# javad-jahangiri-iau/Detecting_Cyber_Attacks_with_Distilled_Large_Language_Models_in_Distributed_Networks

Hardware: AMD Instinct MI355X
Metric: batches/sec/client (DistilBERT seq128 bs32) + aggregated F1 after 1 FedAvg round, 1/2/4/8 MI355X (higher is better)
Workload: dtype bf16; 1 GPU; model=DistilBERT-base (6 layers) + Linear(768,2) DDoSClassifier, global_batch=32, seq_len=128, parallelism=fedavg1 (1 client/GPU)

## Files before the change

csrc/kernels/gemm.hip:

```cpp
#include "common.h"
#include "adam_epi.h"

#include <cstdlib>
#include <cstring>

namespace {

#include "adam_common.h"
#include "attn_s128.h"

enum Epi : int {
  EPI_BF16 = 0,
  EPI_BIAS = 1,
  EPI_BIAS_GELU = 2,
  EPI_GELU_BWD = 3,
  EPI_ADD = 4,
  EPI_F32 = 5,
  EPI_LN = 6,
  EPI_LN_BWD = 7,
  EPI_LN2 = 8,
  EPI_LN2_BWD = 9,
  EPI_F32P = 10,
};
constexpr bool epi_f32(int e) { return e == EPI_F32 || e == EPI_F32P; }

struct GemmParams {
  const bf16_t* A;
  const bf16_t* B;
  void* C;
  int M, N, K;
  int lda, ldb, ldc;
  const float* bias;
  bf16_t* aux;
  int ldaux;
  const bf16_t* res;
  int ldres;
  int k_split;
// ... 38 lines not shown
  }
}
#else
#define FD_STAMP(i) do {} while (0)
DEV void stamp_hwid() {}
#endif

DEV void tile_coords(int lid, int tiles_m, int tiles_n, int gm, int& tm, int& tn) {
  const int per_group = gm * tiles_n;
  const int group = lid / per_group;
  const int first_m = group * gm;
  const int rows = min(gm, tiles_m - first_m);
  const int in_group = lid - group * per_group;
  tm = first_m + in_group % rows;
  tn = in_group / rows;
}

typedef __attribute__((address_space(3))) void lds_void;
typedef __attribute__((address_space(1))) const void gbl_void;

#ifndef FD_GLDS_ASM
#define FD_GLDS_ASM 1
#endif
DEV void glds16(const void* src, char* lds) {
#if FD_GLDS_ASM
  const uint32_t dst = __builtin_amdgcn_readfirstlane(
      (uint32_t)(uintptr_t)(lds_void*)lds);
  uint32_t keep;
  asm volatile("s_mov_b32 %0, m0\n\ts_mov_b32 m0, %2\n\ts_nop 0\n\tglobal_load_lds_dwordx4 %1, off\n\ts_mov_b32 m0, %0"
               : "=&s"(keep) : "v"(src), "s"(dst) : "memory");
#else
  __builtin_amdgcn_global_load_lds((gbl_void*)src, (lds_void*)lds, 16, 0, 0);
#endif
}

template <int W>
DEV int fk(int k) {
  if constexpr (W == 128) return ((k & 3) | ((k >> 1) & 4)) << 1;
  else return (((k >> 1) & 1) | ((k >> 2) & 2)) << 1;
}

DEV int ksw(int r) { return (r >> 1) & 7; }

template <int ROWS, bool KMAJ, int NWAVES, int BK = BKT>
struct Operand {
  static_assert(BK == BKT || (!KMAJ && BK == 32), "32-deep slots: MN-major images only");
  static constexpr int BYTES = ROWS * BK * 2;
  static constexpr int PER_WAVE = BYTES / 1024 / NWAVES;
  static constexpr int SUB = (ROWS % 128 == 0) ? 128 : 64;
  static constexpr int SUB_BYTES = BK * SUB * 2;
  static constexpr int SUB_CH = SUB / 8;

  DEV static void stage(const bf16_t* base, int ld, int row0, int k0, int lim, char* lds, int wid, int lane) {
    const char* sbase = reinterpret_cast<const char*>(KMAJ ? base + k0 : base + (size_t)k0 * ld + row0);
#pragma unroll
    for (int i = 0; i < PER_WAVE; ++i) {
      const int piece = wid * PER_WAVE + i;
      const int pos = piece * 64 + lane;
      uint32_t off;
      if constexpr (KMAJ) {
        const int r = pos >> 3, c = (pos & 7) ^ ksw(r);
        const int gr = min(row0 + r, lim - 1);
        off = (uint32_t)(gr * ld + c * 8) * 2u;
      } else {
        const int sub = pos / (SUB_BYTES / 16), lp = pos % (SUB_BYTES / 16);
        const int k = lp / SUB_CH, c = (lp % SUB_CH) ^ fk<SUB>(k);
// ... 758 lines not shown
  if constexpr (MAXN >= 3) { if (n >= 3) { wait_vm<3 * L>(); return; } }
  if constexpr (MAXN >= 2) { if (n >= 2) { wait_vm<2 * L>(); return; } }
  if constexpr (MAXN >= 1) { if (n >= 1) { wait_vm<L>(); return; } }
  wait_vm<0>();
}

template <int BM, int BN, bool AK, bool BKM, int EPI, int WM, int WN, int S, int BK = BKT>
struct GemmCfg {
  static constexpr int NW = WM * WN;
  using OA = Operand<BM, AK, NW, BK>;
  using OB = Operand<BN, BKM, NW, BK>;
  static constexpr int BUF = OA::BYTES + OB::BYTES;
  static constexpr int EPI_BYTES = EpiTraits<EPI, BM, BN>::DIRECT ? (BM / WM) * (BN * 4 + 16)
                                                                   : EpiTraits<EPI, BM, BN>::BYTES;
  static constexpr int SMEM = S * BUF > EPI_BYTES ? S * BUF : EPI_BYTES;
  static constexpr bool VALID = SMEM <= LDS_MAX && !EpiTraits<EPI, BM, BN>::DIRECT &&
                                (!EpiTraits<EPI, BM, BN>::LN || EpiTraits<EPI, BM, BN>::F32S) &&
                                (BKM || BN % 64 == 0) &&
                                (AK || BM % 64 == 0) &&
                                (BM / WM) % 16 == 0 && (BN / WN) % 16 == 0 &&
                                OA::PER_WAVE * NW * 1024 == OA::BYTES && OB::PER_WAVE * NW * 1024 == OB::BYTES;
};

struct GemmGroup {
  GemmParams q;
  int ntiles0;
  int ntiles;
};

#ifndef FD_GEMM_SCHED
#define FD_GEMM_SCHED 1
#endif

template <int BM, int BN, bool AK, bool BKM, int EPI, int WM, int WN, int S, int BK = BKT, bool WT = false>
DEV void gemm_tile_at(const GemmParams& p, int tm, int tn, char* smem) {
  const int tm_ = tm, tn_ = tn;
  using G = GemmCfg<BM, BN, AK, BKM, EPI, WM, WN, S, BK>;
  constexpr int KS = BK / 32;
  using OA = typename G::OA;
  using OB = typename G::OB;
  constexpr int NW = G::NW;
  constexpr int TM = BM / WM, TN = BN / WN;
  constexpr int MI = TM / 16, NI = TN / 16;
  constexpr int BUF = G::BUF;
  constexpr int L = OA::PER_WAVE + OB::PER_WAVE;
  static_assert(S >= 2 && S <= 6, "ring depth");
  static_assert((S - 2) * L <= 63, "vmcnt is 6 bits");
  constexpr bool SCHED = FD_GEMM_SCHED;

  const int tid = threadIdx.x, lane = tid & 63;
  const int wid = __builtin_amdgcn_readfirstlane(tid >> 6);
  const int wr = wid / WN, wc = wid % WN;
  const int m0 = tm * BM, n0 = tn * BN;
  const int kbeg = blockIdx.z * p.k_split;
  const int nk = p.k_split / BK;

  f32x4 acc[MI][NI];
#pragma unroll
  for (int i = 0; i < MI; ++i)
#pragma unroll
    for (int j = 0; j < NI; ++j) acc[i][j] = f32x4{0.f, 0.f, 0.f, 0.f};

  auto issue = [&](int t) {
    char* b = smem + (t % S) * BUF;
    OA::stage(p.A, p.lda, m0, kbeg + t * BK, p.M, b, wid, lane);
    OB::stage(p.B, p.ldb, n0, kbeg + t * BK, p.N, b + OA::BYTES, wid, lane);
  };
// ... 19 lines not shown
    }
  };
  auto read_frags = [&](const char* cur) {
#pragma unroll
    for (int i = 0; i < MI; ++i) a0[i] = OA::frag(cur, wr * TM + i * 16, 0, lane);
#pragma unroll
    for (int j = 0; j < NI; ++j) b0[j] = OB::frag(cur + OA::BYTES, wc * TN + j * 16, 0, lane);
    if constexpr (KS == 2) {
#pragma unroll
      for (int i = 0; i < MI; ++i) a1[i] = OA::frag(cur, wr * TM + i * 16, 1, lane);
#pragma unroll
      for (int j = 0; j < NI; ++j) b1[j] = OB::frag(cur + OA::BYTES, wc * TN + j * 16, 1, lane);
    }
  };
  auto mfmas = [&]() {
    if constexpr (!SCHED) __builtin_amdgcn_s_setprio(1);
#pragma unroll
    for (int i = 0; i < MI; ++i)
#pragma unroll
      for (int j = 0; j < NI; ++j) acc[i][j] = mfma16(b0[j], a0[i], acc[i][j]);
    if constexpr (KS == 2) {
#pragma unroll
      for (int i = 0; i < MI; ++i)
#pragma unroll
        for (int j = 0; j < NI; ++j) acc[i][j] = mfma16(b1[j], a1[i], acc[i][j]);
    }
    if constexpr (!SCHED) __builtin_amdgcn_s_setprio(0);
  };

  constexpr bool LNPF = EpiTraits<EPI, BM, BN>::LN && S >= 6 && BN == 64 && (BM * BN * 2 / 1024) % NW == 0 &&
                        2 * BUF >= LN_DMA_MISC + 3072;
  const bool lnpf = LNPF && nk % S == 0 && nk >= S && p.M % 4 == 0 && !(p.diag & (1 | 128));
  int e_ops = 0;
  if constexpr (S < 6) {
#pragma unroll
    for (int t = 0; t < S - 1; ++t)
      if (t < nk) issue(t);

    for (int kt = 0; kt < nk; ++kt) {
      wait_tiles<L, S - 2>(min(S - 2, nk - 1 - kt));
      __builtin_amdgcn_s_barrier();
      asm volatile("" ::: "memory");
      if (FD_GEMM_STAMPS && kt == 0) FD_STAMP(1);
      if (kt + S - 1 < nk && !(p.diag & 1)) issue(kt + S - 1);
      read_frags(smem + (kt % S) * BUF);
      mfmas();
      sum_a();
      if constexpr (SCHED) sched_ktile<(MI * (AK ? 1 : 2) + NI * (BKM ? 1 : 2)) * KS / 2, MI * NI * KS / 2>();
    }
  } else {
#pragma unroll
    for (int t = 0; t < S - 2; ++t)
      if (t < nk) issue(t);

    for (int kt = 0; kt < nk; kt += 2) {
      const int issued = min(nk, S - 2 + kt);
      const int need = min(kt + 2, nk);
      if (LNPF && lnpf && kt == nk - 2) {
        wait_ops(e_ops);
      } else {
        wait_tiles<L, S - 4>(min(S - 4, max(0, issued - need)));
      }
      __builtin_amdgcn_s_barrier();
      asm volatile("" ::: "memory");
      if (FD_GEMM_STAMPS && kt == 0) FD_STAMP(1);
      if (!(p.diag & 1)) {
        if (kt + S - 2 < nk) issue(kt + S - 2);
// ... 68 lines not shown
        }
      }
      __syncthreads();
      f32_epilogue<TM, BN, 64 * NW, EPI == EPI_F32P>(p, smem, LDC, m0 + band * TM, n0, tid);
    }
  } else if constexpr (EpiTraits<EPI, BM, BN>::LN2) {
    static_assert((BM == 128 || BM == 256) && BN == 128 && WM == 4 && TN == 64, "two-K-half LayerNorm tile");
    constexpr bool BWD2 = EPI == EPI_LN2_BWD;
    const int s = p.ln2_half, tn_ln = 2 * tn + s, pair = tm * (p.N / BN) + tn;
    const uint32_t tag =
        (uint32_t)__hip_atomic_load(p.ln.cnt, __ATOMIC_RELAXED, __HIP_MEMORY_SCOPE_AGENT) * FD_LN_XSITES + p.ln.xsite + 1u;
    ln2_send<MI, NI>(p, acc, pair, s, wr, wc, lane, tag);
    const auto pre = ln_prefetch<BM, 64, BWD2, 64 * NW>(p, tm, tn_ln, tid);
    ln2_recv<MI, NI>(p, acc, pair, s, wc, wr, lane, tag);
    if (wc == s) ln_park<BM, 64, TM, TN, BWD2>(p, acc, smem, tn_ln * 64, wr, 0, lane);
    ln_finish<BM, 64, BWD2, 64 * NW>(p, smem, tm, tn_ln, lane, tid, pre);
  } else if constexpr (EpiTraits<EPI, BM, BN>::LN) {
    if (LNPF && lnpf) {
      wait_vm<0>();
      __syncthreads();
      const auto pre = ln_from_lds<BM, BN, EPI == EPI_LN_BWD, 64 * NW>(p, tm, tn, tid, smem);
      ln_epilogue<BM, BN, TM, TN, EPI == EPI_LN_BWD, 64 * NW>(p, acc, smem + 2 * BUF, tm, tn, wr, wc, lane, tid, pre);
    } else {
      const auto pre = ln_prefetch<BM, BN, EPI == EPI_LN_BWD, 64 * NW>(p, tm, tn, tid);
      __syncthreads();
      ln_epilogue<BM, BN, TM, TN, EPI == EPI_LN_BWD, 64 * NW>(p, acc, smem, tm, tn, wr, wc, lane, tid, pre);
    }
  } else {
    __syncthreads();
    staged_epilogue<BM, BN, TM, TN, EPI, 64 * NW, WT>(p, acc, smem, m0, n0, wr, wc, lane, tid);
  }
}

template <int BM, int BN, bool AK, bool BKM, int EPI, int WM, int WN, int S, int BK = BKT>
DEV void gemm_tile(const GemmParams& p, int bid, char* smem) {
  int tm, tn;
  tile_coords(bid, (p.M + BM - 1) / BM, p.N / BN, p.group_m, tm, tn);
  gemm_tile_at<BM, BN, AK, BKM, EPI, WM, WN, S, BK>(p, tm, tn, smem);
}

template <int BM, int BN, bool AK, bool BKM, int EPI, int WM, int WN, int S>
__global__ __launch_bounds__(64 * WM * WN, 2) void gemm_kernel(GemmParams p0, GemmGroup grp) {
  using G = GemmCfg<BM, BN, AK, BKM, EPI, WM, WN, S>;
  __shared__ __attribute__((aligned(1024))) char smem[G::SMEM];
  FD_STAMP(0);
  stamp_hwid();
  int bid = xcd_remap(blockIdx.x, grp.ntiles);
  const bool second = bid >= grp.ntiles0;
  const GemmParams& p = second ? grp.q : p0;
  if (second) bid -= grp.ntiles0;
  gemm_tile<BM, BN, AK, BKM, EPI, WM, WN, S>(p, bid, smem);
#if FD_GEMM_STAMPS
  __syncthreads();
  FD_STAMP(5);
#endif
}

struct QkvAttnSync {
  uint64_t* flags;
  const int* cnt;
  int* err;
  int xsite;
  int ntiles, tiles_n;
};
constexpr int QA_BM = 128, QA_BN = 192, QA_NW = 8;
using QaCfg = GemmCfg<QA_BM, QA_BN, true, true, EPI_BIAS, 2, 4, 2>;
static_assert(QaCfg::VALID && QaCfg::NW == QA_NW && QaCfg::SMEM >= ATT_FWD_SMEM, "fused QKV + attention tile");

__global__ __launch_bounds__(64 * QA_NW, 2) void gemm_attn_fwd_kernel(GemmParams p, AttnArgs a, QkvAttnSync q) {
  __shared__ __attribute__((aligned(1024))) char smem[QaCfg::SMEM];
  const uint32_t tag =
// ... 311 lines not shown
  const int lid = xcd_remap(blockIdx.x, gridDim.x);
  const int pair = lid >> 1, s = lid & 1, tiles_n2 = p.N / 128;
  GemmParams q = p;
  const int kh = p.K / 2;
  q.A = p.A + (size_t)s * kh;
  q.B = BKM ? p.B + (size_t)s * kh : p.B + (size_t)s * kh * p.ldb;
  q.k_split = kh;
  q.ln2_half = s;
  gemm_tile_at<BM, 128, true, BKM, EPI, 4, 2, S>(q, pair / tiles_n2, pair % tiles_n2, smem);
#if FD_GEMM_STAMPS
  __syncthreads();
  FD_STAMP(5);
#endif
}

constexpr int DWB_MAXP = 32;
using DwProb = FdDwProb;
struct DwBatch {
  DwProb pr[DWB_MAXP];
  int n, K, ntiles, group_m;
  int diag;
  const int* step;
  float lr, b1, b2, eps, wd;
  int decoupled;
  FdLrSched sched;
  float mu;
  FdAdamRest rest;
  int mixed;
  int cls_tiles[3], cls_off[3], cls_pad[3];
};

constexpr int DWB_HBM = 256, DWB_HBN = 128, DWB_HWM = 4, DWB_HWN = 2;

template <int BM, int BN, int WM, int WN, int S, int BK, bool MIX = false, bool PROX = false>
DEV void dwb_tile(const DwBatch& bt, int lid, char* smem) {
  constexpr int EPI = PROX ? EPI_F32P : EPI_F32;
  int i = 0;
  while (i + 1 < bt.n && lid >= bt.pr[i + 1].tile0) ++i;
  const DwProb& q = bt.pr[i];
  GemmParams p{};
  p.A = q.A; p.B = q.B; p.C = q.C;
  const int K = q.K > 0 ? q.K : bt.K;
  p.M = q.M; p.N = q.N; p.K = K;
  p.lda = q.M; p.ldb = q.N; p.ldc = q.N;
  p.k_split = K;
  p.group_m = bt.group_m;
  p.diag = bt.diag;
  p.out = q.C;
  p.accumulate = q.accumulate;
  p.acol = q.bias;
  if (q.p) {
    p.adam.p = q.p; p.adam.m = q.m; p.adam.v = q.v; p.adam.sh = q.sh; p.adam.step = bt.step;
    p.adam.lr = bt.lr; p.adam.b1 = bt.b1; p.adam.b2 = bt.b2; p.adam.eps = bt.eps; p.adam.wd = q.wd;
    p.adam.decoupled = bt.decoupled;
    if constexpr (PROX) {
      p.adam.mu = bt.mu;
      p.adam.anchor = q.anchor;
    }
    if (bt.sched.kind != 0)
      p.adam.lr = __int_as_float(
          __builtin_amdgcn_readfirstlane(__float_as_int(adam_lr_at(bt.lr, bt.sched, bt.step[0]))));
    if (q.bias && bt.rest.p) {
      const ptrdiff_t off = q.bias - bt.rest.g;
      p.acol_p = bt.rest.p + off; p.acol_m = bt.rest.m + off; p.acol_v = bt.rest.v + off;
      p.acol_sh = bt.rest.sh ? bt.rest.sh + off : nullptr;
      p.acol_wd = q.bias_wd;
      if constexpr (PROX) p.acol_a = bt.rest.anchor ? bt.rest.anchor + off : nullptr;
    }
  }
  if constexpr (MIX) {
    if (q.half) {
      gemm_tile<DWB_HBM, DWB_HBN, false, false, EPI, DWB_HWM, DWB_HWN, S, BK>(p, lid - q.tile0, smem);
      return;
    }
  }
  gemm_tile<BM, BN, false, false, EPI, WM, WN, S, BK>(p, lid - q.tile0, smem);
}

DEV int dwb_mixed_lid(const DwBatch& bt, int b) {
  const int x = b % 8;
  int j = b / 8, c = 0;
  while (c < 2 && j >= bt.cls_pad[c]) {
    j -= bt.cls_pad[c];
    ++c;
  }
  if (j >= bt.cls_pad[c]) return -1;
  const int t = x * bt.cls_pad[c] + j;
  return t < bt.cls_tiles[c] ? bt.cls_off[c] + t : -1;
}

constexpr int DWB_RUNS_LDS = 4096;
template <int NT, bool PROX>
DEV void dwb_rest(const DwBatch& bt, int rb, char* smem) {
  const FdAdamRest& r = bt.rest;
  float lr_t, ss, inv;
  adam_bias_corr(bt.step, bt.lr, bt.sched, bt.b1, bt.b2, lr_t, ss, inv);
  AdamArgs a{};
  a.step = bt.step; a.lr = lr_t; a.b1 = bt.b1; a.b2 = bt.b2; a.eps = bt.eps;
  a.mu = PROX ? bt.mu : 0.f;
  if (rb < r.flat_blocks) {
    a.p = r.p; a.g = r.g; a.m = r.m; a.v = r.v; a.shadow = reinterpret_cast<bf16_t*>(r.sh);
    a.anchor = r.anchor;
    a.wd = bt.wd; a.decoupled = bt.decoupled;
    a.runs = r.runs; a.nruns = r.nruns; a.n4 = r.n4;
    a.run_wd = r.run_wd;
    if (r.runs && 3 * r.nruns <= DWB_RUNS_LDS) {
      long long* rl = reinterpret_cast<long long*>(smem);
      for (int i = threadIdx.x; i < 3 * r.nruns; i += NT) rl[i] = r.runs[i];
      __syncthreads();
// ... 25 lines not shown
        if (v0 + u * stride >= r.n4) continue;
        const long long i = idx[u];
        float pp[4] = {p4[u].x, p4[u].y, p4[u].z, p4[u].w}, gg[4] = {g4[u].x, g4[u].y, g4[u].z, g4[u].w};
        float mm[4] = {m4[u].x, m4[u].y, m4[u].z, m4[u].w}, vv[4] = {v4[u].x, v4[u].y, v4[u].z, v4[u].w};
        adam_math4(a, wd[u], pp, gg, mm, vv, a4[u], ss, inv);
        st_nt(reinterpret_cast<float4*>(a.p) + i, make_float4(pp[0], pp[1], pp[2], pp[3]));
        st_nt(reinterpret_cast<float4*>(a.m) + i, make_float4(mm[0], mm[1], mm[2], mm[3]));
        st_nt(reinterpret_cast<float4*>(a.v) + i, make_float4(vv[0], vv[1], vv[2], vv[3]));
        if (a.shadow)
          reinterpret_cast<uint2*>(a.shadow)[i] = make_uint2(pack_bf2(pp[0], pp[1]), pack_bf2(pp[2], pp[3]));
      }
    }
    return;
  }
  if (!r.ever) return;
  a.p = r.p + r.woff; a.g = r.g + r.woff; a.m = r.m + r.woff; a.v = r.v + r.woff;
  a.shadow = r.sh ? reinterpret_cast<bf16_t*>(r.sh) + r.woff : nullptr;
  a.anchor = r.anchor ? r.anchor + r.woff : nullptr;
  a.wd = r.wwd; a.decoupled = bt.decoupled;
  a.touched = r.ever; a.now = r.now;
  const int lane = threadIdx.x & 63;
  const int nwaves = r.row_blocks * (NT / 64);
  for (int r0 = ((rb - r.flat_blocks) * (NT / 64) + (int)(threadIdx.x >> 6)) * 16; r0 < r.wrows; r0 += nwaves * 16)
    adam_rows16(a, r0, r.wrows, r.wrow4, lane, ss, inv);
}

template <int BM, int BN, int WM, int WN, int S, int BK, bool MIX>
constexpr int dwb_smem() {
  using G = GemmCfg<BM, BN, false, false, EPI_F32, WM, WN, S, BK>;
  using H = GemmCfg<DWB_HBM, DWB_HBN, false, false, EPI_F32, DWB_HWM, DWB_HWN, S, BK>;
  return MIX && H::SMEM > G::SMEM ? H::SMEM : G::SMEM;
}

template <int BM, int BN, int WM, int WN, int S, int BK = BKT, bool MIX = false, bool PROX = false>
__global__ __launch_bounds__(64 * WM * WN, 2) void gemm_dw_batch_kernel(DwBatch bt) {
  constexpr int SMEM = dwb_smem<BM, BN, WM, WN, S, BK, MIX>();
  static_assert(SMEM <= LDS_MAX, "LDS");
  static_assert(!MIX || (BM == DWB_HBM && WM * WN == DWB_HWM * DWB_HWN), "mixed tiles share the block shape");
  __shared__ __attribute__((aligned(1024))) char smem[SMEM];
  const int nrest = bt.rest.flat_blocks + bt.rest.row_blocks;
  int bid = blockIdx.x;
  if (bt.rest.first) {
    if (bid < nrest) {
      dwb_rest<64 * WM * WN, PROX>(bt, bid, smem);
      return;
    }
    bid -= nrest;
  } else {
    const int nblk = MIX && bt.mixed ? 8 * (bt.cls_pad[0] + bt.cls_pad[1] + bt.cls_pad[2]) : bt.ntiles;
    if (bid >= nblk) {
      dwb_rest<64 * WM * WN, PROX>(bt, bid - nblk, smem);
      return;
    }
  }
  if constexpr (MIX) {
    if (bt.mixed) {
      const int lid = dwb_mixed_lid(bt, bid);
      if (lid >= 0) dwb_tile<BM, BN, WM, WN, S, BK, true, PROX>(bt, lid, smem);
      return;
    }
  }
  dwb_tile<BM, BN, WM, WN, S, BK, false, PROX>(bt, xcd_remap(bid, bt.ntiles), smem);
}

__global__ __launch_bounds__(256) void splitk_reduce_kernel(const float* __restrict__ slabs, float* __restrict__ out,
                                                            long long n4, long long stride, int splits,
                                                            int accumulate) {
  for (long long i = blockIdx.x * 256ll + threadIdx.x; i < n4; i += (long long)gridDim.x * 256) {
    float4 s = accumulate ? reinterpret_cast<float4*>(out)[i] : make_float4(0.f, 0.f, 0.f, 0.f);
    for (int z = 0; z < splits; ++z) {
      const float4 v = reinterpret_cast<const float4*>(slabs + z * stride)[i];
      s.x += v.x; s.y += v.y; s.z += v.z; s.w += v.w;
    }
    reinterpret_cast<float4*>(out)[i] = s;
  }
}

constexpr int RED_MAXJ = 16;
struct ReduceJob {
  const float* slabs;
  float* out;
  long long n4, stride;
  int splits, accumulate;
};
struct ReduceBatch {
  ReduceJob j[RED_MAXJ];
  int start[RED_MAXJ + 1];
  int n;
};

__global__ __launch_bounds__(256) void splitk_reduce_batched_kernel(ReduceBatch rb) {
  int ji = 0;
  while (ji + 1 < rb.n && (int)blockIdx.x >= rb.start[ji + 1]) ++ji;
  const ReduceJob& jb = rb.j[ji];
  const int b0 = rb.start[ji], nb = rb.start[ji + 1] - b0;
// ... 411 lines not shown
  const int id = dw2_cfg(M0, N0, M1, N1);
  static const int diag = [] { const char* e = getenv("FD_GEMM_DIAG"); return e ? atoi(e) : 0; }();
  GemmParams p[2]{};
  const void* As[2] = {A0, A1};
  const void* Bs[2] = {B0, B1};
  float* Cs[2] = {C0, C1};
  const int Ms[2] = {M0, M1}, Ns[2] = {N0, N1};
  const long long panel = (long long)CFGS[id].bm * K * 2;
  const int gm = (int)std::max(1ll, std::min(16ll, (2ll << 20) / panel));
  for (int i = 0; i < 2; ++i) {
    p[i].A = (const bf16_t*)As[i]; p[i].B = (const bf16_t*)Bs[i]; p[i].C = Cs[i];
    p[i].M = Ms[i]; p[i].N = Ns[i]; p[i].K = K; p[i].lda = Ms[i]; p[i].ldb = Ns[i]; p[i].ldc = Ns[i];
    p[i].group_m = gm; p[i].diag = diag;
  }
  const int splits = fd_gemm_dw2_splits(M0, N0, M1, N1, K);
  if (splits <= 0) return 6;
  return dw_launch(p, 2, id, splits, K, workspace, workspace_elems, accumulate, adams, defer, splits_out, st);
}

bool dwb_launch_cfg(int id, DwBatch& bt, hipStream_t st, bool dry) {
  auto go = [&](auto kern, int bm, int bn, int threads) {
    for (int i = 0; i < bt.n; ++i)
      if (bt.pr[i].M % bm || bt.pr[i].N % (bt.pr[i].half ? DWB_HBN : bn)) return false;
    int t = 0;
    for (int i = 0; i < bt.n; ++i) {
      bt.pr[i].tile0 = t;
      t += (bt.pr[i].M / bm) * (bt.pr[i].N / (bt.pr[i].half ? DWB_HBN : bn));
    }
    bt.ntiles = t;
    const int nblk = bt.mixed ? 8 * (bt.cls_pad[0] + bt.cls_pad[1] + bt.cls_pad[2]) : t;
    if (!dry) hipLaunchKernelGGL(kern, dim3(nblk + bt.rest.flat_blocks + bt.rest.row_blocks), dim3(threads), 0, st, bt);
    return true;
  };
  if (bt.mixed && id != 11) return false;
  if (bt.mu != 0.f) {
    switch (id) {
      case 1: return go(gemm_dw_batch_kernel<128, 128, 2, 2, 2, BKT, false, true>, 128, 128, 256);
      case 8: return go(gemm_dw_batch_kernel<128, 64, 2, 2, 2, BKT, false, true>, 128, 64, 256);
      case 11: return go(gemm_dw_batch_kernel<256, 256, 2, 4, 2, BKT, true, true>, 256, 256, 512);
    }
    return false;
  }
  switch (id) {
    case 1: return go(gemm_dw_batch_kernel<128, 128, 2, 2, 2>, 128, 128, 256);
    case 8: return go(gemm_dw_batch_kernel<128, 64, 2, 2, 2>, 128, 64, 256);
    case 11: return go(gemm_dw_batch_kernel<256, 256, 2, 4, 2, BKT, true>, 256, 256, 512);
  }
  return false;
}

int g_dwb_mix = -1;
long long g_dwb_mixed_launches = 0;

int dwb_cus() {
  static const int cus = [] {
    int dev = 0, n = 0;
    if (hipGetDevice(&dev) != hipSuccess || hipDeviceGetAttribute(&n, hipDeviceAttributeMultiprocessorCount, dev) !=
                                                 hipSuccess)
      n = 0;
    return n > 0 ? n : 256;
  }();
  return cus;
}

bool plan_dwb_mix(DwBatch& bt, int mode) {
  if (mode <= 0 || bt.n < 2) return false;
  const int cus = dwb_cus();
  int kmax = 0;
  for (int i = 0; i < bt.n; ++i) kmax = std::max(kmax, bt.pr[i].K > 0 ? bt.pr[i].K : bt.K);
  int cls[DWB_MAXP], tiles[DWB_MAXP], L = 0, Sh = 0, nlong = 0;
  for (int i = 0; i < bt.n; ++i) {
    const DwProb& q = bt.pr[i];
    if (q.M % 256 || q.N % 256) return false;
    const int k = q.K > 0 ? q.K : bt.K;
    tiles[i] = (q.M / 256) * (q.N / 256);
    cls[i] = 8 * k <= kmax ? 2 : 0;
    if (cls[i] == 0) { L += tiles[i]; ++nlong; } else Sh += tiles[i];
  }
  if (nlong < 2) return false;
// ... 70 lines not shown
    if (!hyper || !step || !rest->g || !rest->m || !rest->v || (rest->nruns > 0) != (rest->runs != nullptr) ||
        rest->n4 < 0 || (rest->ever && (rest->wrows <= 0 || rest->wrow4 <= 0 || rest->woff % 4)))
      return 7;
    if ((rest->run_wd && !rest->runs) || (rest->ever && rest->wwd != 0.f && hyper[5] == 0.f)) return 8;
    bt.rest = *rest;
    bt.rest.flat_blocks = rest->n4 > 0 ? (int)std::min<long long>(128, (rest->n4 + 2047) / 2048) : 0;
    bt.rest.row_blocks = rest->ever ? std::min(128, (rest->wrows + 127) / 128) : 0;
    static const int first = [] { const char* e = getenv("FD_DW_REST_FIRST"); return e ? atoi(e) : 1; }();
    bt.rest.first = first;
    if (first) {
      const int pad = (8 - (bt.rest.flat_blocks + bt.rest.row_blocks) % 8) % 8;
      bt.rest.row_blocks += pad;
    }
  }
  bt.n = n;
  bt.K = K;
  static const int diag = [] { const char* e = getenv("FD_GEMM_DIAG"); return e ? atoi(e) : 0; }();
  bt.diag = diag;
  for (int i = 0; i < n; ++i) {
    bt.pr[i] = probs[i];
    if (!probs[i].A || !probs[i].B || (!probs[i].C && !probs[i].p) || probs[i].M <= 0 || probs[i].N <= 0) return 2;
    if (probs[i].K < 0 || probs[i].K % BKT) return 5;
    if (probs[i].p && (!probs[i].m || !probs[i].v || !step || !hyper)) return 3;
  }
  if (hyper) {
    bt.step = step;
    bt.lr = hyper[0]; bt.b1 = hyper[1]; bt.b2 = hyper[2]; bt.eps = hyper[3]; bt.wd = hyper[4];
    bt.decoupled = hyper[5] != 0.f;
    if (sched) bt.sched = *sched;
  }
  int id = cfg;
  if (id < 0) {
    static const int env = [] { const char* e = getenv("FD_GEMM_DWB_CFG"); return e ? atoi(e) : -1; }();
    id = env >= 0 ? env : 11;
  }
  bt.group_m = 64;
  static const int gm_env = [] { const char* e = getenv("FD_DWB_GROUP_M"); return e ? atoi(e) : 0; }();
  if (gm_env > 0) bt.group_m = gm_env;
  if (g_dwb_mix < 0) {
    const char* e = getenv("FD_DWB_MIX");
    g_dwb_mix = e ? atoi(e) : 1;
  }
  if (id == 11 && plan_dwb_mix(bt, g_dwb_mix) && !dwb_launch_cfg(id, bt, st, true)) {
    bt.mixed = 0;
    for (int i = 0; i < n; ++i) bt.pr[i] = probs[i];
  }
  if (bt.mixed) ++g_dwb_mixed_launches;
  if (!dwb_launch_cfg(id, bt, st, true)) {
    id = 8;
    if (!dwb_launch_cfg(id, bt, st, true)) return 4;
  }
  dwb_launch_cfg(id, bt, st, false);
  return 0;
}

int fd_splitk_reduce_batched(int n, const float* const* slabs, float* const* outs, const long long* numel,
                             const int* splits, const int* accumulate, hipStream_t st) {
  for (int base = 0; base < n; base += RED_MAXJ) {
    ReduceBatch rb{};
    rb.n = std::min(RED_MAXJ, n - base);
    int blocks = 0;
    for (int i = 0; i < rb.n; ++i) {
      const int k = base + i;
      if (numel[k] % 4 || splits[k] < 1) return 1;
      rb.j[i] = ReduceJob{slabs[k], outs[k], numel[k] / 4, numel[k], splits[k], accumulate[k]};
      rb.start[i] = blocks;
      blocks += (int)std::min<long long>((numel[k] / 4 + 1023) / 1024, 1024);
    }
    rb.start[rb.n] = blocks;
    hipLaunchKernelGGL(splitk_reduce_batched_kernel, dim3(blocks), dim3(256), 0, st, rb);
  }
  return 0;
}


long long fd_gemm_dwb_mixed_launches() { return g_dwb_mixed_launches; }
// ... 88 lines not shown
```

Measured before the change: 653.3 batches/s (sum over clients; bs32 x seq128).

## Add phased half-buffer pipelined main loop for 256x256 weight-gradient batch GEMM

Adds a new main-loop schedule for the 256x256 batched dW GEMM (config 13, now the default). Each K tile is split into four phases that read fragment quadrants and refill 16 KiB half-buffers as soon as their reads retire, with one counted vmcnt wait per tile and staggered barriers between wave rows. It also uses scalar-base global-to-LDS loads. The goal is to overlap DMA with MFMA work inside a two-slot ring without draining the pipeline. In exchange it adds more barriers per tile, a compile-time plan header with static checks, and a host simulator to verify RAW/WAR ordering.

```diff
diff --git a/csrc/host_check/dwb_phase_plan_check.cpp b/csrc/host_check/dwb_phase_plan_check.cpp
--- /dev/null
+++ b/csrc/host_check/dwb_phase_plan_check.cpp
@@ -0,0 +1,130 @@
+#include <cstdio>
+#include <deque>
+#include <vector>
+
+#include "../kernels/dwb_phase_plan.h"
+
+using namespace dwb_plan;
+
+namespace {
+
+constexpr int BIG = 1 << 30;
+enum Mode { STEADY, DRAIN, LAST };
+
+struct Group {
+  int interval = 0;
+  std::deque<int> fifo;
+  void barrier() { ++interval; }
+};
+
+struct Sim {
+  int nk;
+  std::vector<int> issue[2], retired[2], read_done[2];
+  int errors = 0;
+  explicit Sim(int nk_) : nk(nk_) {
+    for (int g = 0; g < 2; ++g) {
+      issue[g].assign(nk * HALVES, -1);
+      retired[g].assign(nk * HALVES, BIG);
+      read_done[g].assign(nk * HALVES, -1);
+    }
+  }
+  void fail(const char* what, int t, int h, int g) {
+    if (errors++ < 8) std::printf("  nk %d: %s (tile %d half %d group %d)\n", nk, what, t, h, g);
+  }
+  void stage(Group& G, int g, int t, int h) {
+    if (issue[g][t * HALVES + h] >= 0) fail("half-buffer staged twice", t, h, g);
+    for (int op = 0; op < OPS_PER_HALF; ++op) G.fifo.push_back(t * HALVES + h);
+    issue[g][t * HALVES + h] = G.interval;
+  }
+  void wait(Group& G, int g, int n) {
+    while ((int)G.fifo.size() > n) {
+      retired[g][G.fifo.front()] = G.interval;
+      G.fifo.pop_front();
+    }
+  }
+  void tile(Group& G, int g, int t, Mode mode) {
+    for (int p = 0; p < PHASES; ++p) {
+      const Phase& ph = PLAN[p];
+      for (int h = 0; h < HALVES; ++h)
+        if ((halves_of(ph.reads) >> h) & 1u) read_done[g][t * HALVES + h] = G.interval + 1;
+      for (int h = 0; h < HALVES; ++h)
+        if ((halves_of(ph.reads) >> h) & 1u) read_at.push_back({t * HALVES + h, g, G.interval});
+      if (mode != LAST)
+        for (int h = 0; h < HALVES; ++h)
+          if ((ph.stage_prev >> h) & 1u) stage(G, g, t + 1, h);
+      if (mode == STEADY)
+        for (int h = 0; h < HALVES; ++h)
+          if ((ph.stage >> h) & 1u) stage(G, g, t + 2, h);
+      if (ph.vmcnt >= 0 && mode != LAST) wait(G, g, mode == STEADY ? ph.vmcnt : 0);
+      G.barrier();
+      G.barrier();
+    }
+  }
+  struct Read { int id, g, interval; };
+  std::vector<Read> read_at;
+
+  int run_group(int g, bool stagger) {
+    Group G;
+    for (int h = 0; h < HALVES; ++h) stage(G, g, 0, h);
+    for (int h = 0; h < HALVES; ++h)
+      if ((own_halves() >> h) & 1u) stage(G, g, 1, h);
+    wait(G, g, PROLOGUE_VMCNT);
+    G.barrier();
+    if (stagger && g == 1) G.barrier();
+    int t = 0;
+    for (; t + 3 < nk; t += 2) {
+      tile(G, g, t, STEADY);
+      tile(G, g, t + 1, STEADY);
+    }
+    if (nk - t == 3) {
+      tile(G, g, t, STEADY);
+      tile(G, g, t + 1, DRAIN);
+      tile(G, g, t + 2, LAST);
+    } else {
+      tile(G, g, t, DRAIN);
+      tile(G, g, t + 1, LAST);
+    }
+    if (stagger && g == 0) G.barrier();
+    if (!G.fifo.empty()) fail("DMA still in flight at the epilogue", -1, -1, g);
+    return G.interval;
+  }
+  bool run(bool stagger) {
+    const int b0 = run_group(0, stagger), b1 = run_group(1, stagger);
+    if (b0 != b1 || b0 != 1 + BARRIERS_PER_TILE * nk + (stagger ? 1 : 0)) fail("barrier counts differ", -1, -1, 0);
+    for (const Read& r : read_at) {
+      const int t = r.id / HALVES, h = r.id % HALVES;
+      for (int g = 0; g < 2; ++g) {
+        if (issue[g][r.id] < 0) fail("read of a half-buffer that was never staged", t, h, g);
+        if (r.interval <= retired[g][r.id]) fail("RAW: read not behind the barrier after the retiring wait", t, h, r.g);
+      }
+    }
+    for (int id = 2 * HALVES; id < nk * HALVES; ++id)
+      for (int gi = 0; gi < 2; ++gi)
+        for (int gr = 0; gr < 2; ++gr)
+          if (issue[gi][id] <= read_done[gr][id - 2 * HALVES]) fail("WAR: refill not behind the reads' barrier", id / HALVES, id % HALVES, gi);
+    for (int t = 0; t < nk; ++t)
+      for (int h = 0; h < HALVES; ++h)
+        for (int g = 0; g < 2; ++g)
+          if (read_done[g][t * HALVES + h] < 0) fail("half-buffer never read", t, h, g);
+    return errors == 0;
+  }
+};
+
+}
+
+int main() {
+  bool ok = true;
+  const int nks[] = {2, 3, 4, 5, 6, 7, 8, 41, 42};
+  for (int nk : nks)
+    for (int stagger = 0; stagger < 2; ++stagger) {
+      Sim s(nk);
+      if (!s.run(stagger != 0)) {
+        std::printf("nk %d stagger %d: FAILED\n", nk, stagger);
+        ok = false;
+      }
+    }
+  std::printf("steady vmcnt %d, prologue vmcnt %d, barriers per K tile %d\n", STEADY_VMCNT, PROLOGUE_VMCNT,
+              BARRIERS_PER_TILE);
+  std::printf(ok ? "dwb phase plan check: ok\n" : "dwb phase plan check: FAILED\n");
+  return ok ? 0 : 1;
+}
diff --git a/csrc/kernels/dwb_phase_plan.h b/csrc/kernels/dwb_phase_plan.h
--- /dev/null
+++ b/csrc/kernels/dwb_phase_plan.h
@@ -0,0 +1,124 @@
+#pragma once
+
+namespace dwb_plan {
+
+constexpr int PHASES = 4;
+constexpr int HALVES = 4;
+constexpr int OPS_PER_HALF = 2;
+constexpr int HALF_BYTES = 16384;
+constexpr int WAR_GAP = 2;
+
+enum : unsigned { RD_ALO = 1, RD_AHI = 2, RD_BLO = 4, RD_BHI = 8 };
+enum : unsigned { H_A0 = 1, H_A1 = 2, H_B0 = 4, H_B1 = 8 };
+
+struct Phase {
+  unsigned reads;
+  int qi, qj;
+  unsigned stage_prev;
+  unsigned stage;
+  int vmcnt;
+};
+
+constexpr Phase PLAN[PHASES] = {
+    {RD_ALO | RD_BLO, 0, 0, H_A0 | H_A1, 0, -1},
+    {RD_BHI, 0, 1, 0, 0, -1},
+    {RD_AHI, 1, 1, 0, 0, -1},
+    {0, 1, 0, 0, H_B0 | H_B1, 4},
+};
+
+constexpr unsigned halves_of(unsigned reads) {
+  return ((reads & (RD_ALO | RD_AHI)) ? (H_A0 | H_A1) : 0u) | ((reads & (RD_BLO | RD_BHI)) ? (H_B0 | H_B1) : 0u);
+}
+constexpr int popcount(unsigned x) { return x ? int(x & 1u) + popcount(x >> 1) : 0; }
+constexpr unsigned frags_of(int qi, int qj) { return (qi ? RD_AHI : RD_ALO) | (qj ? RD_BHI : RD_BLO); }
+
+constexpr int wait_phase() {
+  for (int p = 0; p < PHASES; ++p)
+    if (PLAN[p].vmcnt >= 0) return p;
+  return -1;
+}
+constexpr int last_read_phase(unsigned half) {
+  int r = -1;
+  for (int p = 0; p < PHASES; ++p)
+    if (halves_of(PLAN[p].reads) & half) r = p;
+  return r;
+}
+constexpr int first_read_phase() {
+  for (int p = 0; p < PHASES; ++p)
+    if (PLAN[p].reads) return p;
+  return -1;
+}
+
+constexpr bool covers() {
+  unsigned quads = 0, have = 0;
+  for (int p = 0; p < PHASES; ++p) {
+    const Phase& ph = PLAN[p];
+    if (ph.qi < 0 || ph.qi > 1 || ph.qj < 0 || ph.qj > 1) return false;
+    if (have & ph.reads) return false;
+    have |= ph.reads;
+    if ((have & frags_of(ph.qi, ph.qj)) != frags_of(ph.qi, ph.qj)) return false;
+    const unsigned q = 1u << (2 * ph.qi + ph.qj);
+    if (quads & q) return false;
+    quads |= q;
+  }
+  return quads == 15u && have == 15u;
+}
+constexpr unsigned own_halves() {
+  unsigned m = 0;
+  for (int p = 0; p < PHASES; ++p) m |= PLAN[p].stage;
+  return m;
+}
+constexpr unsigned prev_halves() {
+  unsigned m = 0;
+  for (int p = 0; p < PHASES; ++p) m |= PLAN[p].stage_prev;
+  return m;
+}
+constexpr bool stages_once() {
+  unsigned seen = 0;
+  bool own_seen = false;
+  for (int p = 0; p < PHASES; ++p) {
+    if (PLAN[p].stage_prev && own_seen) return false;
+    if (seen & (PLAN[p].stage | PLAN[p].stage_prev) || (PLAN[p].stage & PLAN[p].stage_prev)) return false;
+    seen |= PLAN[p].stage | PLAN[p].stage_prev;
+    own_seen = own_seen || PLAN[p].stage;
+  }
+  return seen == 15u;
+}
+constexpr bool war_ok() {
+  for (int p = 0; p < PHASES; ++p)
+    for (int h = 0; h < HALVES; ++h) {
+      if ((PLAN[p].stage >> h) & 1u)
+        if (p < last_read_phase(1u << h) + WAR_GAP) return false;
+      if ((PLAN[p].stage_prev >> h) & 1u)
+        if (p + PHASES < last_read_phase(1u << h) + WAR_GAP) return false;
+    }
+  return true;
+}
+constexpr int ops_in_flight_at_wait() {
+  int n = 0;
+  for (int p = 0; p <= wait_phase(); ++p) n += popcount(PLAN[p].stage) * OPS_PER_HALF;
+  return n;
+}
+constexpr bool raw_ok() {
+  int waits = 0;
+  for (int p = 0; p < PHASES; ++p) waits += PLAN[p].vmcnt >= 0;
+  if (waits != 1) return false;
+  const int pw = wait_phase();
+  for (int p = pw + 1; p < PHASES; ++p)
+    if (PLAN[p].stage_prev) return false;
+  if (PLAN[pw].vmcnt != ops_in_flight_at_wait()) return false;
+  return PHASES + first_read_phase() - pw >= 1;
+}
+
+constexpr int PROLOGUE_VMCNT = popcount(own_halves()) * OPS_PER_HALF;
+constexpr int STEADY_VMCNT = PLAN[wait_phase() < 0 ? 0 : wait_phase()].vmcnt;
+constexpr int MIN_NK = 2;
+constexpr int BARRIERS_PER_TILE = 2 * PHASES;
+
+static_assert(covers(), "each accumulator quadrant once, each fragment set read once and before its use");
+static_assert(stages_once(), "each half-buffer is refilled exactly once per K tile");
+static_assert(war_ok(), "a half-buffer is refilled >= WAR_GAP phases after its last fragment read");
+static_assert(raw_ok(), "one counted wait per K tile; it retires tile t + 1 one phase or more before its first read");
+static_assert(STEADY_VMCNT > 0 && STEADY_VMCNT <= 63, "the steady-state wait is counted (vmcnt is 6 bits)");
+
+}
diff --git a/csrc/kernels/gemm.hip b/csrc/kernels/gemm.hip
--- a/csrc/kernels/gemm.hip
+++ b/csrc/kernels/gemm.hip
@@ -1,8 +1,10 @@
 #include "common.h"
 #include "adam_epi.h"
+#include "dwb_phase_plan.h"
 
 #include <cstdlib>
 #include <cstring>
+#include <type_traits>
 
 namespace {
 
@@ -107,6 +109,12 @@
 #else
   __builtin_amdgcn_global_load_lds((gbl_void*)src, (lds_void*)lds, 16, 0, 0);
 #endif
+}
+
+DEV void glds16s(const void* sbase, uint32_t off, uint32_t dst) {
+  uint32_t keep;
+  asm volatile("s_mov_b32 %0, m0\n\ts_mov_b32 m0, %2\n\ts_nop 0\n\tglobal_load_lds_dwordx4 %1, %3\n\ts_mov_b32 m0, %0"
+               : "=&s"(keep) : "v"(off), "s"(dst), "s"(sbase) : "memory");
 }
 
 template <int W>
@@ -931,7 +939,7 @@
 #define FD_GEMM_SCHED 1
 #endif
 
-template <int BM, int BN, bool AK, bool BKM, int EPI, int WM, int WN, int S, int BK = BKT, bool WT = false>
+template <int BM, int BN, bool AK, bool BKM, int EPI, int WM, int WN, int S, int BK = BKT, bool WT = false, bool PH = false>
 DEV void gemm_tile_at(const GemmParams& p, int tm, int tn, char* smem) {
   const int tm_ = tm, tn_ = tn;
   using G = GemmCfg<BM, BN, AK, BKM, EPI, WM, WN, S, BK>;
@@ -1017,7 +1025,147 @@
                         2 * BUF >= LN_DMA_MISC + 3072;
   const bool lnpf = LNPF && nk % S == 0 && nk >= S && p.M % 4 == 0 && !(p.diag & (1 | 128));
   int e_ops = 0;
-  if constexpr (S < 6) {
+  bool ring = true;
+  if constexpr (PH) {
+    namespace pl = dwb_plan;
+    static_assert(BM == 256 && BN == 256 && WM == 2 && WN == 4 && S == 2 && BK == 64 && !AK && !BKM,
+                  "the phased loop is written for the 256 x 256 MN-major tile on 2 x 4 waves, two 64 KiB slots");
+    static_assert(OA::SUB_BYTES == pl::HALF_BYTES && OA::BYTES == 2 * pl::HALF_BYTES && BUF == pl::HALVES * pl::HALF_BYTES &&
+                      pl::HALF_BYTES / 1024 == NW * pl::OPS_PER_HALF && MI == 8 && NI == 4,
+                  "four 16 KiB half-buffers per slot (A0 A1 B0 B1), 2 pieces per wave per half-buffer");
+    if (nk >= pl::MIN_NK) {
+      ring = false;
+      uint32_t offA[pl::OPS_PER_HALF], offB[pl::OPS_PER_HALF];
+#pragma unroll
+      for (int i = 0; i < pl::OPS_PER_HALF; ++i) {
+        const int lp = (wid * pl::OPS_PER_HALF + i) * 64 + lane;
+        const int k = lp / OA::SUB_CH, c = (lp % OA::SUB_CH) ^ fk<128>(k);
+        offA[i] = (uint32_t)(k * p.lda + c * 8) * 2u;
+        offB[i] = (uint32_t)(k * p.ldb + c * 8) * 2u;
+      }
+      const char* gA = reinterpret_cast<const char*>(p.A + (size_t)kbeg * p.lda + m0);
+      const char* gB = reinterpret_cast<const char*>(p.B + (size_t)kbeg * p.ldb + n0);
+      const size_t stepA = (size_t)BK * p.lda * 2, stepB = (size_t)BK * p.ldb * 2;
+      auto half_at = [&](int h, int sl) { return smem + (2 * h + sl) * pl::HALF_BYTES; };
+      const uint32_t lds0 = __builtin_amdgcn_readfirstlane((uint32_t)(uintptr_t)(lds_void*)smem) +
+                            (uint32_t)wid * (pl::OPS_PER_HALF * 1024);
+      auto stage_half = [&](int h, int t, int sl) {
+        const char* src = (h >= 2 ? gB + t * stepB : gA + t * stepA) + (h & 1) * (OA::SUB * 2);
+        const uint32_t dst = lds0 + (uint32_t)(2 * h + sl) * pl::HALF_BYTES;
+#pragma unroll
+        for (int i = 0; i < pl::OPS_PER_HALF; ++i) glds16s(src, h >= 2 ? offB[i] : offA[i], dst + i * 1024);
+      };
+      const char* const aimg = half_at(wr, 0);
+      const char* const bimg = half_at(2 + wc / 2, 0);
+      auto read_a = [&](int sl, int ih) {
+#pragma unroll
+        for (int i = 4 * ih; i < 4 * ih + 4; ++i) {
+          a0[i] = OA::frag(aimg + sl * pl::HALF_BYTES, i * 16, 0, lane);
+          a1[i] = OA::frag(aimg + sl * pl::HALF_BYTES, i * 16, 1, lane);
+        }
+      };
+      auto read_b = [&](int sl, int jh) {
+#pragma unroll
+        for (int j = 2 * jh; j < 2 * jh + 2; ++j) {
+          b0[j] = OB::frag(bimg + sl * pl::HALF_BYTES, (wc % 2) * TN + j * 16, 0, lane);
+          b1[j] = OB::frag(bimg + sl * pl::HALF_BYTES, (wc % 2) * TN + j * 16, 1, lane);
+        }
+      };
+      auto sum_a_half = [&](int ih) {
+        if (acs) {
+#pragma unroll
+          for (int i = 4 * ih; i < 4 * ih + 4; ++i) {
+            float s = 0.f;
+#pragma unroll
+            for (int e = 0; e < 8; ++e) {
+              s += bf2f((uint16_t)a0[i][e]);
+              s += bf2f((uint16_t)a1[i][e]);
+            }
+            asum[i] += s;
+          }
+        }
+      };
+      auto phase = [&](auto pc, auto mc, auto sc, int t) {
+        constexpr int P = decltype(pc)::value, MODE = decltype(mc)::value, cur = decltype(sc)::value;
+        constexpr pl::Phase ph = pl::PLAN[P];
+        if constexpr ((ph.reads & pl::RD_BLO) != 0) read_b(cur, 0);
+        if constexpr ((ph.reads & pl::RD_BHI) != 0) read_b(cur, 1);
+        if constexpr ((ph.reads & pl::RD_ALO) != 0) read_a(cur, 0);
+        if constexpr ((ph.reads & pl::RD_AHI) != 0) read_a(cur, 1);
+        if constexpr (ph.stage_prev != 0) {
+          if ((MODE == 0 || t + 1 < nk) && !(p.diag & 1)) {
+#pragma unroll
+            for (int h = 0; h < pl::HALVES; ++h)
+              if ((ph.stage_prev >> h) & 1u) stage_half(h, t + 1, cur ^ 1);
+          }
+        }
+        if constexpr (ph.stage != 0) {
+          if ((MODE == 0 || t + 2 < nk) && !(p.diag & 1)) {
+#pragma unroll
+            for (int h = 0; h < pl::HALVES; ++h)
+              if ((ph.stage >> h) & 1u) stage_half(h, t + 2, cur);
+          }
+        }
+        if constexpr (ph.vmcnt >= 0) {
+          if (MODE == 0 || t + 2 < nk) wait_vm<ph.vmcnt>();
+          else if (t + 1 < nk) wait_vm<0>();
+        }
+        asm volatile("" ::: "memory");
+        __builtin_amdgcn_s_barrier();
+        asm volatile("s_waitcnt lgkmcnt(0)" ::: "memory");
+        __builtin_amdgcn_sched_barrier(0);
+        __builtin_amdgcn_s_setprio(1);
+#pragma unroll
+        for (int i = 4 * ph.qi; i < 4 * ph.qi + 4; ++i)
+#pragma unroll
+          for (int j = 2 * ph.qj; j < 2 * ph.qj + 2; ++j) acc[i][j] = mfma16(b0[j], a0[i], acc[i][j]);
+#pragma unroll
+        for (int i = 4 * ph.qi; i < 4 * ph.qi + 4; ++i)
+#pragma unroll
+          for (int j = 2 * ph.qj; j < 2 * ph.qj + 2; ++j) acc[i][j] = mfma16(b1[j], a1[i], acc[i][j]);
+        __builtin_amdgcn_s_setprio(0);
+        if constexpr ((ph.reads & pl::RD_ALO) != 0) sum_a_half(0);
+        if constexpr ((ph.reads & pl::RD_AHI) != 0) sum_a_half(1);
+        __builtin_amdgcn_sched_barrier(0);
+        __builtin_amdgcn_s_barrier();
+        asm volatile("" ::: "memory");
+      };
+      auto ktile = [&](auto mc, auto cur, int t) {
+        phase(std::integral_constant<int, 0>{}, mc, cur, t);
+        phase(std::integral_constant<int, 1>{}, mc, cur, t);
+        phase(std::integral_constant<int, 2>{}, mc, cur, t);
+        phase(std::integral_constant<int, 3>{}, mc, cur, t);
+      };
+      constexpr std::integral_constant<int, 0> STEADY{};
+      constexpr std::integral_constant<int, 1> TAIL{};
+      constexpr std::integral_constant<int, 0> s0{};
+      constexpr std::integral_constant<int, 1> s1{};
+
+#pragma unroll
+      for (int h = 0; h < pl::HALVES; ++h) stage_half(h, 0, 0);
+#pragma unroll
+      for (int h = 0; h < pl::HALVES; ++h)
+        if ((pl::own_halves() >> h) & 1u) stage_half(h, 1, 1);
+      wait_vm<pl::PROLOGUE_VMCNT>();
+      asm volatile("" ::: "memory");
+      __builtin_amdgcn_s_barrier();
+      asm volatile("" ::: "memory");
+      FD_STAMP(1);
+      if (wr == 1) __builtin_amdgcn_s_barrier();
+      int t = 0;
+      for (; t + 3 < nk; t += 2) {
+        ktile(STEADY, s0, t);
+        ktile(STEADY, s1, t + 1);
+      }
+      for (; t < nk; t += 2) {
+        ktile(TAIL, s0, t);
+        if (t + 1 < nk) ktile(TAIL, s1, t + 1);
+      }
+      if (wr == 0) __builtin_amdgcn_s_barrier();
+    }
+  }
+  if (!ring) {
+  } else if constexpr (S < 6) {
 #pragma unroll
     for (int t = 0; t < S - 1; ++t)
       if (t < nk) issue(t);
@@ -1152,11 +1300,11 @@
   }
 }
 
-template <int BM, int BN, bool AK, bool BKM, int EPI, int WM, int WN, int S, int BK = BKT>
+template <int BM, int BN, bool AK, bool BKM, int EPI, int WM, int WN, int S, int BK = BKT, bool PH = false>
 DEV void gemm_tile(const GemmParams& p, int bid, char* smem) {
   int tm, tn;
   tile_coords(bid, (p.M + BM - 1) / BM, p.N / BN, p.group_m, tm, tn);
-  gemm_tile_at<BM, BN, AK, BKM, EPI, WM, WN, S, BK>(p, tm, tn, smem);
+  gemm_tile_at<BM, BN, AK, BKM, EPI, WM, WN, S, BK, false, PH>(p, tm, tn, smem);
 }
 
 template <int BM, int BN, bool AK, bool BKM, int EPI, int WM, int WN, int S>
@@ -1534,7 +1682,7 @@
 
 constexpr int DWB_HBM = 256, DWB_HBN = 128, DWB_HWM = 4, DWB_HWN = 2;
 
-template <int BM, int BN, int WM, int WN, int S, int BK, bool MIX = false, bool PROX = false>
+template <int BM, int BN, int WM, int WN, int S, int BK, bool MIX = false, bool PROX = false, bool PH = false>
 DEV void dwb_tile(const DwBatch& bt, int lid, char* smem) {
   constexpr int EPI = PROX ? EPI_F32P : EPI_F32;
   int i = 0;
@@ -1576,7 +1724,7 @@
       return;
     }
   }
-  gemm_tile<BM, BN, false, false, EPI, WM, WN, S, BK>(p, lid - q.tile0, smem);
+  gemm_tile<BM, BN, false, false, EPI, WM, WN, S, BK, PH>(p, lid - q.tile0, smem);
 }
 
 DEV int dwb_mixed_lid(const DwBatch& bt, int b) {
@@ -1668,7 +1816,7 @@
   return MIX && H::SMEM > G::SMEM ? H::SMEM : G::SMEM;
 }
 
-template <int BM, int BN, int WM, int WN, int S, int BK = BKT, bool MIX = false, bool PROX = false>
+template <int BM, int BN, int WM, int WN, int S, int BK = BKT, bool MIX = false, bool PROX = false, bool PH = false>
 __global__ __launch_bounds__(64 * WM * WN, 2) void gemm_dw_batch_kernel(DwBatch bt) {
   constexpr int SMEM = dwb_smem<BM, BN, WM, WN, S, BK, MIX>();
   static_assert(SMEM <= LDS_MAX, "LDS");
@@ -1692,11 +1840,25 @@
   if constexpr (MIX) {
     if (bt.mixed) {
       const int lid = dwb_mixed_lid(bt, bid);
-      if (lid >= 0) dwb_tile<BM, BN, WM, WN, S, BK, true, PROX>(bt, lid, smem);
+      if (lid >= 0) {
+        FD_STAMP(0);
+        stamp_hwid();
+        dwb_tile<BM, BN, WM, WN, S, BK, true, PROX, PH>(bt, lid, smem);
+#if FD_GEMM_STAMPS
+        __syncthreads();
+        FD_STAMP(5);
+#endif
+      }
       return;
     }
   }
-  dwb_tile<BM, BN, WM, WN, S, BK, false, PROX>(bt, xcd_remap(bid, bt.ntiles), smem);
+  FD_STAMP(0);
+  stamp_hwid();
+  dwb_tile<BM, BN, WM, WN, S, BK, false, PROX, PH>(bt, xcd_remap(bid, bt.ntiles), smem);
+#if FD_GEMM_STAMPS
+  __syncthreads();
+  FD_STAMP(5);
+#endif
 }
 
 __global__ __launch_bounds__(256) void splitk_reduce_kernel(const float* __restrict__ slabs, float* __restrict__ out,
@@ -2174,12 +2336,13 @@
     if (!dry) hipLaunchKernelGGL(kern, dim3(nblk + bt.rest.flat_blocks + bt.rest.row_blocks), dim3(threads), 0, st, bt);
     return true;
   };
-  if (bt.mixed && id != 11) return false;
+  if (bt.mixed && id != 11 && id != 13) return false;
   if (bt.mu != 0.f) {
     switch (id) {
       case 1: return go(gemm_dw_batch_kernel<128, 128, 2, 2, 2, BKT, false, true>, 128, 128, 256);
       case 8: return go(gemm_dw_batch_kernel<128, 64, 2, 2, 2, BKT, false, true>, 128, 64, 256);
       case 11: return go(gemm_dw_batch_kernel<256, 256, 2, 4, 2, BKT, true, true>, 256, 256, 512);
+      case 13: return go(gemm_dw_batch_kernel<256, 256, 2, 4, 2, BKT, true, true, true>, 256, 256, 512);
     }
     return false;
   }
@@ -2187,6 +2350,7 @@
     case 1: return go(gemm_dw_batch_kernel<128, 128, 2, 2, 2>, 128, 128, 256);
     case 8: return go(gemm_dw_batch_kernel<128, 64, 2, 2, 2>, 128, 64, 256);
     case 11: return go(gemm_dw_batch_kernel<256, 256, 2, 4, 2, BKT, true>, 256, 256, 512);
+    case 13: return go(gemm_dw_batch_kernel<256, 256, 2, 4, 2, BKT, true, false, true>, 256, 256, 512);
   }
   return false;
 }
@@ -2323,7 +2487,7 @@
   int id = cfg;
   if (id < 0) {
     static const int env = [] { const char* e = getenv("FD_GEMM_DWB_CFG"); return e ? atoi(e) : -1; }();
-    id = env >= 0 ? env : 11;
+    id = env >= 0 ? env : 13;
   }
   bt.group_m = 64;
   static const int gm_env = [] { const char* e = getenv("FD_DWB_GROUP_M"); return e ? atoi(e) : 0; }();
@@ -2332,7 +2496,7 @@
     const char* e = getenv("FD_DWB_MIX");
     g_dwb_mix = e ? atoi(e) : 1;
   }
-  if (id == 11 && plan_dwb_mix(bt, g_dwb_mix) && !dwb_launch_cfg(id, bt, st, true)) {
+  if ((id == 11 || id == 13) && plan_dwb_mix(bt, g_dwb_mix) && !dwb_launch_cfg(id, bt, st, true)) {
     bt.mixed = 0;
     for (int i = 0; i < n; ++i) bt.pr[i] = probs[i];
   }
```

New measurement: 658.7 batches/s (sum over clients; bs32 x seq128), median of 6. Within noise of the previous version (+0.8%).
